# librosa/librosa

Hardware: AMD Instinct MI355X
Metric: STFT+mel frames/sec (n_fft=2048 hop=512) (higher is better)
Workload: dtype f32

## Files before the change

include/librosa_amd.h:

```cpp
#ifndef LIBROSA_AMD_H
#define LIBROSA_AMD_H

#include <stddef.h>
#include <stdint.h>

#ifdef __cplusplus
extern "C" {
#endif

#define LRA_OK 0
#define LRA_EINVAL (-1)
#define LRA_EHIP (-2)
#define LRA_EROCFFT (-3)
#define LRA_ENODEV (-4)
#define LRA_ENOMEM (-5)

#define LRA_F32 0
#define LRA_F64 1

#define LRA_PAD_CONSTANT 0
#define LRA_PAD_REFLECT 1
#define LRA_PAD_EDGE 2
#define LRA_PAD_SYMMETRIC 3

// ... 176 lines not shown
    int halve;
    int64_t n;
    const void* row_ptr;
    const void* col;
    const void* val;
} lra_cqt_octave;
int lra_cqt_recursion_exec(lra_ctx* ctx, const void* y, int64_t batch, const lra_cqt_octave* octaves, int n_octaves, int pad_mode, const void* sqrt_len, void* out, int64_t n_frames,
                           int n_total, const void* taps, int n_taps, int first, void* scratch, int64_t scratch_bytes, int overlap, int dtype);
int lra_cqt_octave_exec(lra_ctx* ctx, const void* y, int64_t batch, int64_t n, int64_t y_stride, int n_fft, int hop, int pad_mode, const void* row_ptr, const void* col, const void* val,
                        const void* sqrt_len, void* out, int64_t n_frames, int n_total, int bin0, int row0, int n_rows, int dtype);

int lra_magnitude_exec(lra_ctx* ctx, const void* D, void* mag, int64_t count, int dtype);

int lra_magphase_exec(lra_ctx* ctx, const void* D, int is_complex, void* mag, void* phase, int64_t count, double power, int dtype);

int lra_hpss_exec(lra_ctx* ctx, const void* mag, const void* D, void* out_h, void* out_p, int64_t batch, int64_t n_frames, int n_bins, int win_harm, int win_perc, double power,
                  double margin_harm, double margin_perc, int want_mask, int dtype);

#define LRA_COMM_ID_BYTES 128
typedef struct lra_comm lra_comm;
int lra_comm_unique_id(void* id_out);
int lra_comm_init(lra_ctx* ctx, int rank, int n_ranks, const void* id, lra_comm** out);
int lra_comm_allgather(lra_comm* comm, const void* send_dev, void* recv_dev, size_t bytes_per_rank);
int lra_comm_allgatherv(lra_comm* comm, const void* send_dev, void* recv_dev, const size_t* bytes_per_rank, const size_t* recv_offsets);
void lra_comm_destroy(lra_comm* comm);

int lra_probe_stream(lra_ctx* ctx, int direction, const void* in, void* out, int64_t batch, int64_t rows_per_clip, int n_fft, int hop, int64_t clip_samples,
                     int strip_rows, int waves_per_cu);
int lra_probe_stream_pitched(lra_ctx* ctx, int direction, const void* in, void* out, int64_t batch, int64_t rows_per_clip, int n_fft, int hop, int64_t clip_samples,
                             int strip_rows, int waves_per_cu, int64_t row_pitch_bytes, int piece_bytes);

int lra_probe_stream_window(lra_ctx* ctx, const void* in, void* out, int64_t batch, int64_t rows_per_clip, int n_fft, int hop, int64_t clip_samples, int strip_rows, int waves_per_cu);

int lra_transpose(lra_ctx* ctx, const void* src, void* dst, int64_t batch, int64_t rows, int64_t cols, int elem_bytes);

#ifdef __cplusplus
}
#endif
#endif
```

librosa_amd/_native.py:

```python
from __future__ import annotations

import collections
import ctypes
import os
import threading
from ctypes import POINTER, byref, c_char_p, c_double, c_float, c_int, c_int64, c_size_t, c_void_p

import numpy as np

from .util.exceptions import LibrosaError, ParameterError

_HERE = os.path.dirname(os.path.abspath(__file__))
LIB_PATH = os.environ.get("LIBROSA_AMD_LIBRARY") or os.path.join(_HERE, "_liblibrosa_amd.so")

LRA_OK, LRA_EINVAL, LRA_EHIP, LRA_EROCFFT, LRA_ENODEV, LRA_ENOMEM = 0, -1, -2, -3, -4, -5
LRA_F32, LRA_F64 = 0, 1
PAD_MODES = {"constant": 0, "reflect": 1, "edge": 2, "symmetric": 3}


class NativeError(LibrosaError):
    """The HIP library is missing, or a HIP / rocFFT call failed."""


SIGNATURES = {
# ... 11 lines not shown
    "lra_ctx_nonfinite_reset": (c_int, [c_void_p]),
    "lra_ctx_nonfinite_read": (c_int, [c_void_p, POINTER(c_int)]),
    "lra_stft_plan_is_fused": (c_int, [c_void_p]),
    "lra_stft_plan_tuned_variant": (c_int, [c_void_p, c_int]),
    "lra_istft_plan_tuned_variant": (c_int, [c_void_p]),
    "lra_malloc": (c_int, [c_void_p, c_size_t, POINTER(c_void_p)]),
    "lra_free": (c_int, [c_void_p, c_void_p]),
    "lra_malloc_placed": (c_int, [c_void_p, c_size_t, c_int, c_int64, c_int, POINTER(c_void_p), POINTER(c_float), POINTER(c_int)]),
    "lra_free_placed": (c_int, [c_void_p, c_void_p]),
    "lra_memset": (c_int, [c_void_p, c_void_p, c_int, c_size_t]),
    "lra_memcpy_h2d": (c_int, [c_void_p, c_void_p, c_void_p, c_size_t]),
    "lra_memcpy_d2h": (c_int, [c_void_p, c_void_p, c_void_p, c_size_t]),
    "lra_event_create": (c_int, [c_void_p, POINTER(c_void_p)]),
    "lra_event_destroy": (None, [c_void_p]),
    "lra_event_record": (c_int, [c_void_p]),
    "lra_event_elapsed_ms": (c_int, [c_void_p, c_void_p, POINTER(c_float)]),
    "lra_stft_plan_create": (c_int, [c_void_p, c_int, c_int, c_void_p, c_int, c_int, c_int, POINTER(c_void_p)]),
    "lra_stft_plan_destroy": (None, [c_void_p]),
    "lra_stft_num_frames": (c_int, [c_void_p, c_int64, POINTER(c_int64)]),
    "lra_stft_exec": (c_int, [c_void_p, c_void_p, c_int64, c_int64, c_int64, c_void_p]),
    "lra_spectrogram_exec": (c_int, [c_void_p, c_void_p, c_int64, c_int64, c_int64, c_double, c_void_p]),
    "lra_mel_plan_create": (c_int, [c_void_p, c_int, c_int, c_void_p, c_int, POINTER(c_void_p)]),
    "lra_mel_plan_destroy": (None, [c_void_p]),
    "lra_melspectrogram_exec": (c_int, [c_void_p, c_void_p, c_void_p, c_int64, c_int64, c_int64, c_double, c_void_p]),
    "lra_mel_apply_exec": (c_int, [c_void_p, c_void_p, c_int64, c_int64, c_int64, c_int64, c_int64, c_void_p]),
    "lra_istft_plan_create": (c_int, [c_void_p, c_int, c_int, c_void_p, c_int, c_int, POINTER(c_void_p)]),
    "lra_istft_plan_destroy": (None, [c_void_p]),
    "lra_istft_exec": (c_int, [c_void_p, c_void_p, c_int64, c_int64, c_int64, c_int64, c_void_p, c_void_p, c_int64, c_int64]),
    "lra_istft_exec_norm": (c_int, [c_void_p, c_void_p, c_int64, c_int64, c_int64, c_int64, c_void_p, c_void_p, c_int64, c_int64]),
    "lra_transpose": (c_int, [c_void_p, c_void_p, c_void_p, c_int64, c_int64, c_int64, c_int]),
    "lra_probe_stream": (c_int, [c_void_p, c_int, c_void_p, c_void_p, c_int64, c_int64, c_int, c_int, c_int64, c_int, c_int]),
    "lra_cqt_recursion_exec": (c_int, [c_void_p, c_void_p, c_int64, c_void_p, c_int, c_int, c_void_p, c_void_p, c_int64, c_int, c_void_p, c_int, c_int, c_void_p, c_int64, c_int, c_int]),
    "lra_probe_stream_window": (c_int, [c_void_p, c_void_p, c_void_p, c_int64, c_int64, c_int, c_int, c_int64, c_int, c_int]),
    "lra_pcg64_random_exec": (c_int, [c_void_p, POINTER(ctypes.c_uint64), ctypes.c_uint64, c_void_p, c_int64]),
    "lra_griffinlim_init_pcg64": (c_int, [c_void_p, POINTER(ctypes.c_uint64), c_void_p, c_void_p, c_int64, c_int, c_int64, c_int]),
    "lra_probe_stream_pitched": (c_int, [c_void_p, c_int, c_void_p, c_void_p, c_int64, c_int64, c_int, c_int, c_int64, c_int, c_int, c_int64, c_int]),
    "lra_stft_exec_strided": (c_int, [c_void_p, c_int, c_void_p, c_int64, c_int64, c_int64, c_double, c_void_p, c_int64]),
    "lra_item_absmax_exec": (c_int, [c_void_p, c_void_p, c_int64, c_int64, c_int, c_void_p]),
    "lra_item_max_exec": (c_int, [c_void_p, c_void_p, c_int64, c_int64, c_int, c_int, c_void_p]),
    "lra_to_db_exec": (c_int, [c_void_p, c_void_p, c_void_p, c_int64, c_int64, c_int, c_int, c_double, c_double, c_void_p, c_void_p, c_int, c_double]),
    "lra_from_db_exec": (c_int, [c_void_p, c_void_p, c_void_p, c_int64, c_int, c_int, c_double]),
    "lra_istft_exec_host": (c_int, [c_void_p, c_void_p, c_int64, c_int64, c_int64, c_void_p, c_void_p, c_int64, c_int64]),
    "lra_stft_exec_host": (c_int, [c_void_p, c_void_p, c_int, c_void_p, c_int64, c_int64, c_int64, c_double, c_void_p, c_int64, POINTER(c_int)]),
    "lra_comm_unique_id": (c_int, [c_void_p]),
    "lra_comm_init": (c_int, [c_void_p, c_int, c_int, c_void_p, POINTER(c_void_p)]),
    "lra_comm_allgather": (c_int, [c_void_p, c_void_p, c_void_p, c_size_t]),
    "lra_comm_allgatherv": (c_int, [c_void_p, c_void_p, c_void_p, POINTER(c_size_t), POINTER(c_size_t)]),
    "lra_comm_destroy": (None, [c_void_p]),
    "lra_phase_vocoder_exec": (c_int, [c_void_p, c_void_p, c_void_p, c_int64, c_int64, c_int, c_void_p, c_int64, c_int]),
    "lra_griffinlim_init": (c_int, [c_void_p, c_void_p, c_void_p, c_void_p, c_int64, c_int]),
    "lra_griffinlim_update": (c_int, [c_void_p, c_void_p, c_void_p, c_void_p, c_void_p, c_int64, c_int, c_double, c_double, c_int]),
    "lra_pcen_exec": (c_int, [c_void_p, c_void_p, c_void_p, c_void_p, c_int64, c_int64, c_int, c_double, c_double, c_double, c_double, c_double, c_void_p, c_double, c_void_p]),
    "lra_maxfilter_exec": (c_int, [c_void_p, c_void_p, c_void_p, c_int64, c_int, c_int64, c_int, c_int]),
    "lra_onset_exec": (c_int, [c_void_p, c_void_p, c_void_p, c_void_p, c_int64, c_int, c_int64, c_int, c_int, c_int, c_int, c_void_p, c_void_p, c_int, c_int, c_int64, c_int64, c_int,
                               c_double, c_double, c_void_p, c_int, c_void_p]),
    "lra_beat_work_bytes": (c_int64, [c_int64, c_int64, c_int]),
    "lra_beat_exec": (c_int, [c_void_p, c_void_p, c_int64, c_int64, c_int, c_void_p, c_int, c_double, c_double, c_int, c_void_p, c_void_p, POINTER(c_int)]),
    "lra_peak_pick_work_bytes": (c_int64, [c_int64, c_int64, c_int]),
    "lra_peak_pick_exec": (c_int, [c_void_p, c_void_p, c_int64, c_int64, c_int, c_int, c_int64, c_int64, c_int64, c_int64, c_double, c_int64, c_int, c_void_p, c_void_p, c_void_p,
                                   POINTER(c_int)]),
    "lra_prev_minimum_exec": (c_int, [c_void_p, c_void_p, c_int64, c_int64, c_int, c_void_p]),
    "lra_tempogram_work_bytes": (c_int64, [c_int64, c_int64, c_int, c_int]),
    "lra_tempogram_exec": (c_int, [c_void_p, c_void_p, c_int64, c_int64, c_int, c_int, c_int, c_void_p, c_int, c_int, c_void_p, c_void_p, c_void_p, c_void_p, POINTER(c_int)]),
    "lra_fir_decimate_exec": (c_int, [c_void_p, c_void_p, c_void_p, c_int64, c_int64, c_int64, c_void_p, c_int, c_int, c_int, c_double, c_double, c_int]),
    "lra_resample_poly_exec": (c_int, [c_void_p, c_void_p, c_void_p, c_int64, c_int64, c_int64, c_void_p, c_int, c_int, c_int, c_int, c_double, c_double, c_int]),
    "lra_resample_fft_exec": (c_int, [c_void_p, c_void_p, c_void_p, c_int64, c_int64, c_int64, c_double, c_int]),
# ... 626 lines not shown
```

librosa_amd/csrc/lra_api.hip:

```cpp
#include <dlfcn.h>
#include <hip/hip_runtime.h>
#include <rocfft/rocfft.h>

#include <algorithm>
#include <atomic>
#include <chrono>
#include <cmath>
#include <cstdio>
#include <cstdlib>
#include <cstring>
#include <map>
#include <memory>
#include <mutex>
#include <string>
#include <thread>
#include <vector>

#include "../../include/librosa_amd.h"
#define LRA_FUSED_EXTERN
#include "lra_fused.h"
#include "lra_mel.h"
#include "lra_post.h"
#include "lra_pcen.h"
#include "lra_onset.h"
// ... 368 lines not shown
                const double fill = (v2 && Cfg::TF == 64 && rounds <= 1.0 && rounds >= 0.6) ? 1.0 : rounds / std::ceil(rounds);
                if (fill > best_fill + 0.02) { best_fill = fill; best_iters = it; }
            }
            iters = best_iters;
            while (iters > 4 && batch * ((a.n_frames + fpb * iters - 1) / (fpb * iters)) < 2LL * n_cu) iters /= 2;
        }
        if (iters < 1) iters = 1;
        a.rot_uniform = 0;
        if (Cfg::FPB > 1 && Cfg::TF < 64 && ring_rows_aligned<Cfg>(a.hop)) {
            if (iters_opt <= 0 && iters >= 4) iters = (iters + 3) / 4 * 4;
            a.rot_uniform = iters % 4 == 0;
        }
        a.mel_tile = mel_tile_opt > 0 ? mel_tile_opt : 4;
        if (a.mel_tile > iters) a.mel_tile = iters;
        a.frames_per_wg = Cfg::FPB * iters;
        a.wg_per_clip = (a.n_frames + a.frames_per_wg - 1) / a.frames_per_wg;
        a.slot_bytes = v2 ? stft2_slot_bytes<Cfg>() : direct ? Cfg::FRAME_BYTES : stft_slot_bytes<Cfg>(MODE, a.n_mels, a.mel_tile);
        a.shared_off = Cfg::FPB * a.slot_bytes;
        const long long grid = batch * a.wg_per_clip;
        if (grid > 0x7ffffff0LL) { err = hipErrorInvalidConfiguration; return; }
        const int lds = Cfg::FPB * a.slot_bytes + shared_bytes + lds_pad;
        if (lds > 160 * 1024) { err = hipErrorInvalidValue; return; }
        if (lds > 65536) {
            err = hipFuncSetAttribute(reinterpret_cast<const void*>(kern), hipFuncAttributeMaxDynamicSharedMemorySize, lds);
            if (err != hipSuccess) return;
        }
        a.n_blocks = (int)grid;
        a.xcd_chunk = (xcd_remap && grid >= 64) ? (int)((grid + 7) / 8) : 0;
        const long long launch_grid = a.xcd_chunk ? 8LL * a.xcd_chunk : grid;
        hipLaunchKernelGGL(kern, dim3((unsigned)launch_grid), dim3(Cfg::NT), lds, stream, a, a.y, out);
        err = hipGetLastError();
    }

    template <class Cfg> void launch_pc(int hd) {
        using PL = PcLayout<Cfg>;
        void (*kern)(StftArgs<T>, const T*, void*) = nullptr;
#define LRA_PICKP(HD)                                                        \
    kern = stft_pc_kernel<Cfg, HD, POW_TWO>;                                 \
    if (a.power_mode == POW_ONE) kern = stft_pc_kernel<Cfg, HD, POW_ONE>;    \
    if (a.power_mode == POW_GENERAL) kern = stft_pc_kernel<Cfg, HD, POW_GENERAL>;
        if (hd == 4) { LRA_PICKP(4) } else { LRA_PICKP(8) }
#undef LRA_PICKP
        const int lds = PL::BYTES + lds_pad;
        constexpr int fpb = PL::NP;
        int iters = iters_opt;
        if (iters <= 0) {
            const int per_cu = resident_workgroups(reinterpret_cast<const void*>(kern), PL::NT, lds);
            const long long conc = (long long)n_cu * (per_cu > 0 ? per_cu : 1);
            int best_iters = 0;
            double best_fill = -1.0;
            for (int cand = 176; cand >= 24; --cand) {
                const int wgpc = (a.n_frames + fpb * cand - 1) / (fpb * cand);
                const int it = (a.n_frames + fpb * wgpc - 1) / (fpb * wgpc);
                const double rounds = (double)(batch * wgpc) / (double)conc;
                const double fill = (rounds <= 1.0 && rounds >= 0.6) ? 1.0 : rounds / std::ceil(rounds);
                if (fill > best_fill + 0.02) { best_fill = fill; best_iters = it; }
            }
            iters = best_iters;
            while (iters > 4 && batch * ((a.n_frames + fpb * iters - 1) / (fpb * iters)) < 2LL * n_cu) iters /= 2;
        }
        if (iters < 1) iters = 1;
        a.rot_uniform = 0;
        a.mel_tile = 1;
        a.frames_per_wg = fpb * iters;
        a.wg_per_clip = (a.n_frames + a.frames_per_wg - 1) / a.frames_per_wg;
        a.slot_bytes = PL::FRAME;
        a.shared_off = 0;
        const long long grid = batch * a.wg_per_clip;
        if (grid > 0x7ffffff0LL) { err = hipErrorInvalidConfiguration; return; }
        a.n_blocks = (int)grid;
        a.xcd_chunk = (xcd_remap && grid >= 64) ? (int)((grid + 7) / 8) : 0;
        const long long launch_grid = a.xcd_chunk ? 8LL * a.xcd_chunk : grid;
        hipLaunchKernelGGL(kern, dim3((unsigned)launch_grid), dim3(PL::NT), lds, stream, a, a.y, out);
        err = hipGetLastError();
    }

    template <class Cfg> void operator()() {
        if constexpr (Cfg::REV) {
            err = hipErrorInvalidValue;
            return;
        } else if constexpr (Cfg::PLAN == 1) {
            if (!use_v2 || v2_hop_divisor<Cfg>(a.hop) == 0) { err = hipErrorInvalidValue; return; }
            if (mode == OUT_COMPLEX) launch<Cfg, OUT_COMPLEX>(0);
            else if (mode == OUT_POWER) launch<Cfg, OUT_POWER>(0);
            else if (mode == OUT_MEL2 && mel_pc && mel && mel->melr2_ok && mel_runs) {
                if constexpr (pc_cfg_ok<Cfg>()) {
                    const int hd_pc = v2_hop_divisor<Cfg>(a.hop);
                    if (!pc_bank_ok<Cfg>(a.n_mels, mel->melr2_pmax) || !pc_fits_budget<Cfg>(hd_pc, a.power_mode)) { err = hipErrorInvalidValue; return; }
                    a.melr_w = (const T*)mel->d_melr2_w;
                    a.melr_keep = (const T*)mel->d_melr2_keep;
                    a.melr_addr = mel->d_melr2_addr;
                    a.melr_zero = mel->melr2_zero;
                    a.melr_mid = mel->melr2_mid;
                    a.melr_pmax = mel->melr2_pmax;
                    launch_pc<Cfg>(hd_pc);
                } else err = hipErrorInvalidValue;
            } else err = hipErrorInvalidValue;
        } else {
            run<Cfg>();
        }
    }
    template <class Cfg> void run() {
        if (mode == OUT_MEL2) {
            using MC = typename MelCfgOf<Cfg>::type;
            if constexpr (pc_cfg_ok<Cfg>()) {
                const int hd_pc = v2_hop_divisor<Cfg>(a.hop);
                if (mel_pc && mel && mel->melr2_ok && mel_runs && use_v2 && pc_bank_ok<Cfg>(a.n_mels, mel->melr2_pmax) && pc_fits_budget<Cfg>(hd_pc, a.power_mode)) {
                    a.melr_w = (const T*)mel->d_melr2_w;
                    a.melr_keep = (const T*)mel->d_melr2_keep;
                    a.melr_addr = mel->d_melr2_addr;
                    a.melr_zero = mel->melr2_zero;
                    a.melr_mid = mel->melr2_mid;
                    a.melr_pmax = mel->melr2_pmax;
                    launch_pc<Cfg>(hd_pc);
                    return;
                }
            }
            if constexpr (v2_cfg_ok<MC>()) {
                if (mel && mel->melr2_ok && mel_runs && use_v2 && melr_fits<MC>() && v2_hop_divisor<MC>(a.hop) > 0) {
                    const int shared_r = melr_shared_bytes<MC>(a.n_mels, mel->melr2_pmax);
                    if (MC::FPB * stft2_slot_bytes<MC>() + shared_r <= 160 * 1024) {
                        a.melr_w = (const T*)mel->d_melr2_w;
                        a.melr_keep = (const T*)mel->d_melr2_keep;
                        a.melr_addr = mel->d_melr2_addr;
                        a.melr_zero = mel->melr2_zero;
                        a.melr_mid = mel->melr2_mid;
                        a.melr_pmax = mel->melr2_pmax;
                        mel_v2 = true;
                        mel_tile_opt = 1;
                        launch<MC, OUT_MELR>(shared_r);
                        return;
                    }
                }
            }
            if constexpr (mel_many_applies<Cfg>()) {
                using MM = typename MelManyCfgOf<Cfg>::type;
                if (mel && mel->melr_ok && mel->melr_many && mel_runs && melr_fits<MM>()) {
                    const int shared_m = melr_shared_bytes<MM>(a.n_mels, mel->melr_pmax);
                    if (MM::FPB * stft_slot_bytes<MM>(OUT_MELR, a.n_mels, 1) + shared_m <= 160 * 1024) {
                        a.melr_w = (const T*)mel->d_melr_w;
                        a.melr_keep = (const T*)mel->d_melr_keep;
                        a.melr_addr = mel->d_melr_addr;
                        a.melr_zero = mel->melr_zero;
                        a.melr_mid = mel->melr_mid;
                        a.melr_pmax = mel->melr_pmax;
                        mel_tile_opt = 1;
                        launch<MM, OUT_MELR>(shared_m);
                        return;
// ... 3234 lines not shown
    if (n_fft < 256 || n_fft > 2048 || M % 128 != 0) return fail(LRA_EINVAL, "probe: n_fft must be 256 ... 2048, a multiple of 256");
    if (hop <= 0 || hop > 1024 || hop % 128 != 0) return fail(LRA_EINVAL, "probe: hop must be a multiple of 128, at most 1024");
    if (direction != 0 && direction != 1) return fail(LRA_EINVAL, "probe: direction 0 (forward stream) or 1 (inverse stream)");
    if (rows_per_clip > 0x7fffffffLL || batch > 0x7fffffffLL) return fail(LRA_EINVAL, "probe: too many rows");
    ProbeArgs a;
    a.in = (const char*)in;
    a.out = (char*)out;
    a.clip_in_bytes = (long long)clip_samples * 4;
    a.rows_per_clip = (int)rows_per_clip;
    a.strip_rows = strip_rows > 0 ? strip_rows : 162;
    a.n_clips = (int)batch;
    a.bins = M + 1;
    a.row_pitch = row_pitch_bytes > 0 ? row_pitch_bytes : (long long)(M + 1) * 8;
    if (a.row_pitch < (long long)(M + 1) * 8 || a.row_pitch % 8 != 0) return fail(LRA_EINVAL, "probe: row pitch must be a multiple of 8 bytes, at least one row");
    if (piece_bytes != 8 && piece_bytes != 16) return fail(LRA_EINVAL, "probe: pieces of 8 or 16 bytes");
    if (piece_bytes == 16 && (a.row_pitch % 16 != 0 || ((size_t)(direction == 0 ? out : in) & 15))) return fail(LRA_EINVAL, "probe: 16-byte pieces need 16-byte aligned rows");
    a.hop_bytes = hop * 4;
    const long long pcm_rows = clip_samples / hop;
    a.pcm_rows = (int)(pcm_rows < rows_per_clip ? pcm_rows : rows_per_clip);
    const long long strips = (long long)batch * ((rows_per_clip + a.strip_rows - 1) / a.strip_rows);
    const long long grid = (strips + 7) / 8 * 8;
    if (grid > 0x7ffffff0LL) return fail(LRA_EINVAL, "probe: grid too large");
    a.xcd_chunk = ctx->opt_xcd_remap ? (int)(grid / 8) : 0;
    const int wpc = waves_per_cu > 0 ? waves_per_cu : 12;
    const int lds = wpc >= 32 ? 0 : ((160 * 1024 / wpc) & ~255);
    auto kern = direction == 0 ? (piece_bytes == 16 ? stream_probe_kernel<0, true> : stream_probe_kernel<0, false>)
                               : (piece_bytes == 16 ? stream_probe_kernel<1, true> : stream_probe_kernel<1, false>);
    if (lds > 65536) LRA_HIP(hipFuncSetAttribute(reinterpret_cast<const void*>(kern), hipFuncAttributeMaxDynamicSharedMemorySize, lds));
    hipLaunchKernelGGL(kern, dim3((unsigned)grid), dim3(64), lds, ctx->stream, a);
    LRA_HIP(hipGetLastError());
    return LRA_OK;
}

int lra_probe_stream_window(lra_ctx* ctx, const void* in, void* out, int64_t batch, int64_t rows_per_clip, int n_fft, int hop, int64_t clip_samples, int strip_rows, int waves_per_cu) {
    LRA_BIND(ctx);
    if (batch <= 0 || rows_per_clip <= 0) return LRA_OK;
    if (!in || !out) return fail(LRA_EINVAL, "null data pointer");
    const int M = n_fft / 2;
    if (n_fft < 256 || n_fft > 2048 || M % 128 != 0) return fail(LRA_EINVAL, "probe: n_fft must be 256 ... 2048, a multiple of 256");
    if (hop <= 0 || hop > 1024 || hop % 128 != 0) return fail(LRA_EINVAL, "probe: hop must be a multiple of 128, at most 1024");
    if (strip_rows < 1 || waves_per_cu < 1 || waves_per_cu > 32) return fail(LRA_EINVAL, "probe: strip_rows >= 1, 1 <= waves_per_cu <= 32");
    ProbeArgs a;
    a.in = (const char*)in;
    a.out = (char*)out;
    a.clip_in_bytes = (long long)clip_samples * 4;
    a.rows_per_clip = (int)rows_per_clip;
    a.strip_rows = strip_rows;
    a.n_clips = (int)batch;
    a.bins = M + 1;
    a.row_pitch = (long long)(M + 1) * 8;
    a.hop_bytes = hop * 4;
    const long long pcm_rows = clip_samples / hop;
    a.pcm_rows = (int)(pcm_rows < rows_per_clip ? pcm_rows : rows_per_clip);
    a.xcd_chunk = 0;
    const int n_workers = ctx->n_cu * waves_per_cu;
    const int lds = waves_per_cu >= 32 ? 0 : ((160 * 1024 / waves_per_cu) & ~255);
    if (lds > 65536) LRA_HIP(hipFuncSetAttribute(reinterpret_cast<const void*>(stream_probe_window_kernel), hipFuncAttributeMaxDynamicSharedMemorySize, lds));
    hipLaunchKernelGGL(stream_probe_window_kernel, dim3((unsigned)n_workers), dim3(64), lds, ctx->stream, a, (long long)batch * rows_per_clip, n_workers);
    LRA_HIP(hipGetLastError());
    return LRA_OK;
}

int lra_transpose(lra_ctx* ctx, const void* src, void* dst, int64_t batch, int64_t rows, int64_t cols, int elem_bytes) {
    LRA_BIND(ctx);
    if (batch <= 0 || rows <= 0 || cols <= 0) return LRA_OK;
    if (!src || !dst) return fail(LRA_EINVAL, "null data pointer");
// ... 15 lines not shown
```

librosa_amd/csrc/lra_fused.h:

```cpp
#pragma once

#include <hip/hip_runtime.h>

#include "lra_dispatch.h"
#include "lra_kernels_pc.h"

template <class Cfg, int MODE, int PM, int RA>
__global__ __launch_bounds__(Cfg::NT, Cfg::MIN_WAVES) void stft_kernel(lra::StftArgs<typename Cfg::real> a, const typename Cfg::real* __restrict__ y,
                                                                     void* __restrict__ out) {
    extern __shared__ __attribute__((aligned(16))) char lra_smem[];
    lra::Lds lds;
    lds.base = lra_smem;
    a.y = y;
    a.D = static_cast<typename Cfg::cplx*>(out);
    a.S = static_cast<typename Cfg::real*>(out);
    a.Mel = static_cast<typename Cfg::real*>(out);
    const int blk = lra::xcd_block((int)blockIdx.x, a.xcd_chunk);
    if (blk >= a.n_blocks) return;
    lra::stft_block<Cfg, MODE, PM, RA>(a, blk, lds);
}

constexpr int kV3Waves = 3;
template <class Cfg, int HD, int MODE, int PM>
__global__ __launch_bounds__(Cfg::NT, (Cfg::NT > 256 ? 1 : (Cfg::TF == 64 && HD >= 4 && PM != lra::POW_GENERAL && MODE != lra::OUT_MELR ? (Cfg::PLAN == 1 ? kV3Waves : 3) : 2))) void stft2_kernel(lra::StftArgs<typename Cfg::real> a, const typename Cfg::real* __restrict__ y,
                                                                                  void* __restrict__ out) {
    extern __shared__ __attribute__((aligned(16))) char lra_smem[];
    lra::Lds lds;
    lds.base = lra_smem;
    a.y = y;
    a.D = static_cast<typename Cfg::cplx*>(out);
    a.S = static_cast<typename Cfg::real*>(out);
    a.Mel = static_cast<typename Cfg::real*>(out);
    const int blk = lra::xcd_block((int)blockIdx.x, a.xcd_chunk);
    if (blk >= a.n_blocks) return;
    lra::stft_block2<Cfg, HD, MODE, PM>(a, blk, lds);
}

template <class Cfg, int HD, int PM>
__global__ __launch_bounds__(lra::PcLayout<Cfg>::NT, 3) void stft_pc_kernel(lra::StftArgs<typename Cfg::real> a, const typename Cfg::real* __restrict__ y, void* __restrict__ out) {
    extern __shared__ __attribute__((aligned(32))) char lra_smem[];
    lra::Lds lds;
    lds.base = lra_smem;
    a.y = y;
    a.Mel = static_cast<typename Cfg::real*>(out);
    const int blk = lra::xcd_block((int)blockIdx.x, a.xcd_chunk);
    if (blk >= a.n_blocks) return;
    lra::stft_pc_block<Cfg, HD, PM>(a, blk, lds);
}

template <class Cfg, int HC>
__global__ __launch_bounds__(Cfg::NT, Cfg::MIN_WAVES) void istft_kernel(lra::IstftArgs<typename Cfg::real> a, const typename Cfg::cplx* __restrict__ D,
                                                                      const typename Cfg::real* __restrict__ wss, typename Cfg::real* __restrict__ y) {
    extern __shared__ __attribute__((aligned(16))) char lra_smem[];
    lra::Lds lds;
    lds.base = lra_smem;
    a.D = D;
    a.wss = wss;
    a.y = y;
    const int blk = lra::xcd_block((int)blockIdx.x, a.xcd_chunk);
    if (blk >= a.n_blocks) return;
    lra::istft_block<Cfg, HC>(a, blk, lds);
}


namespace lra {

#define LRA_CFG_ALIAS(NAME, ...) using NAME = typename CfgSel<__VA_ARGS__>::type; using NAME##_mel = typename MelCfgOf<NAME>::type; using NAME##_melmany = typename MelManyCfgOf<NAME>::type;
LRA_CFG_ALIAS(cfg_f32_4, float, 4, 0)
LRA_CFG_ALIAS(cfg_f32_5, float, 5, 0)
LRA_CFG_ALIAS(cfg_f32_6, float, 6, 0)
LRA_CFG_ALIAS(cfg_f32_7, float, 7, 0)
LRA_CFG_ALIAS(cfg_f32_8, float, 8, 0)
LRA_CFG_ALIAS(cfg_f32_9, float, 9, 0)
LRA_CFG_ALIAS(cfg_f32_10, float, 10, 0)
LRA_CFG_ALIAS(cfg_f32_10v1, float, 10, 1)
LRA_CFG_ALIAS(cfg_f32_10v4, float, 10, 4)
LRA_CFG_ALIAS(cfg_f32_10r, float, 10, 5)
LRA_CFG_ALIAS(cfg_f32_10g, float, 10, 6)
LRA_CFG_ALIAS(cfg_f32_10q, float, 10, 7)
LRA_CFG_ALIAS(cfg_f32_11, float, 11, 0)
// ... 74 lines not shown
```

librosa_amd/csrc/lra_kernels_pc.h:

```cpp
#pragma once

#include "lra_kernels2.h"

namespace lra {

constexpr int kPcPrioPA = 3, kPcPrioPS = 2, kPcPrioCA = 0, kPcPrioCB = 1;
constexpr int kPcSpinLimit = 1 << 22;

template <class Cfg> struct PcLayout {
    using T = typename Cfg::real;
    static constexpr int NP = 2;
    static constexpr int NT = (NP + 1) * Cfg::TF;
    static constexpr int FRAME = Cfg::FRAME_BYTES;
    static constexpr int PW = (v2_pw_bytes<Cfg>() + 15) / 16 * 16;
    static constexpr int RS = ((Cfg::R * (Cfg::TF + kMelRsPitchExtra) + 2) * 2 * (int)sizeof(T) + 15) / 16 * 16;
    static constexpr int frame_off(int s) { return s * FRAME; }
    static constexpr int pw_off(int s) { return NP * FRAME + s * PW; }
    static constexpr int rs_off() { return NP * (FRAME + PW); }
    static constexpr int flags_off() { return rs_off() + RS; }
    static constexpr int ready_off(int s) { return flags_off() + 4 * s; }
    static constexpr int consumed_off(int s) { return flags_off() + 4 * (NP + s); }
    static constexpr int BYTES = flags_off() + 16;
};

template <class Cfg> constexpr bool pc_cfg_ok() { return v23_cfg_ok<Cfg>() && Cfg::TF == 64 && v2_pw_swz<Cfg>() && melr_fits<Cfg>() && sizeof(typename Cfg::real) == 4; }
template <class Cfg> LRA_HD bool pc_bank_ok(int n_mels, int pmax) { return n_mels >= 1 && n_mels <= 2 * Cfg::TF && pmax <= 4; }

template <class Cfg> LRA_HD bool pc_fits_budget(int hd, int power_mode) {
    if (power_mode != POW_TWO && power_mode != POW_ONE) return false;
    if (hd == 8) return true;
    return hd == 4 && (power_mode == POW_TWO || Cfg::PLAN == 1);
}

#ifdef LRA_HOSTSIM
struct PcTileV {
    float e[16];
    float& operator[](int i) { return e[i]; }
    float operator[](int i) const { return e[i]; }
};
#else
typedef float PcTileV __attribute__((ext_vector_type(16)));
#endif

template <class Cfg> struct PcRegs {
    using T = typename Cfg::real;
    using C = typename Cfg::cplx;
    static constexpr int NB = 2, PH = 4, TILE = 8, NP = PcLayout<Cfg>::NP;
    C w[Cfg::R];
    C wq;
    T keep[Cfg::R];
    T pw[Cfg::R], pw_extra;
    int mad[NB][2 * PH];
    int pwa[4], pwx;
    T* row[NB];
    int ph[NP][NB];
    PcTileV mt[NP];
// ... 15 lines not shown
}
#endif
template <class T, int MT> LRA_HD void pc_tile_band(const PcTileV& t, int b, T (&out)[MT]) {
    LRA_UNROLL
    for (int k = 0; k < MT; ++k) out[k] = t[MT * b + k];
}

#ifdef LRA_HOSTSIM
LRA_HD int pc_flag_load(Lds l, int off) { return lds_ld<int>(l, off); }
LRA_HD void pc_flag_store(Lds l, int off, int v) { lds_st<int>(l, off, v); }
LRA_HD void pc_wait(Lds, int, int, unsigned int*) {}
LRA_HD void pc_fence() {}
#else
__device__ __forceinline__ void pc_fence() {
    __builtin_amdgcn_fence(__ATOMIC_RELEASE, "wavefront");
    __builtin_amdgcn_wave_barrier();
    __builtin_amdgcn_fence(__ATOMIC_ACQUIRE, "wavefront");
}
__device__ __forceinline__ int pc_flag_load(Lds l, int off) { return *(const volatile __attribute__((address_space(3))) int*)(l.base + off); }
__device__ __forceinline__ void pc_flag_store(Lds l, int off, int v) { *(volatile __attribute__((address_space(3))) int*)(l.base + off) = v; }
__device__ __forceinline__ void pc_wait(Lds l, int off, int want, unsigned int* sticky) {
    int spins = 0;
    while (true) {
        const int v = LRA_UNIFORM(pc_flag_load(l, off));
        if (LRA_LIKELY(v >= want)) break;
        if (LRA_UNLIKELY(++spins > kPcSpinLimit)) {
            if (sticky && (threadIdx.x & 63) == 0) atomicOr(sticky, 2u);
            break;
        }
        __builtin_amdgcn_s_sleep(2);
    }
    pc_fence();
}
__device__ __forceinline__ void pc_wait_ready(Lds l, int off, int want, unsigned int* sticky) {
    if (LRA_UNLIKELY(LRA_UNIFORM(pc_flag_load(l, off)) < want)) pc_wait(l, off, want, sticky);
    else pc_fence();
}
#endif

template <class Cfg, int HD> LRA_HD void pc_producer_prologue(const StftArgs<typename Cfg::real>& a, int clip, int frame0, int tf, Regs2<Cfg, HD>& rg) {
    using T = typename Cfg::real;
    if constexpr (Cfg::PLAN == 1) v3_hoist<Cfg, HD>(rg, tf, a.win, a.tw, a.twr);
    else v2_hoist<Cfg, HD>(rg, tf, a.win, a.tw, a.twr);
    v2_fill<Cfg, HD>(a, clip, frame0, tf, rg);
    if constexpr (v2_rotate_asm_ok<Cfg, HD>()) {
        LRA_UNROLL
        for (int e = 0; e < Cfg::R; ++e) { LRA_KEEP(rg.raw[e].x); LRA_KEEP(rg.raw[e].y); }
    }
    LRA_UNROLL
    for (int e = 0; e < Regs2<Cfg, HD>::NEW; ++e) rg.pf[e] = mk<T>((T)0, (T)0);
}
template <class Cfg, int HD> LRA_HD void pc_producer_pass0(const StftArgs<typename Cfg::real>& a, int clip, int frame, int it, bool more, int tf, Regs2<Cfg, HD>& rg, Lds fr) {
    if (v2_rotate_asm_ok<Cfg, HD>()) {
        v2_window_rotating<Cfg, HD>(it, rg);
        if (more) v2_issue_loads<Cfg, HD>(a, clip, frame + 1, tf, rg);
        v2_pass0_dft<Cfg, HD>(tf, rg, fr);
    } else {
        if (it > 0) v2_shift<Cfg, HD>(rg);
        if (more) v2_issue_loads<Cfg, HD>(a, clip, frame + 1, tf, rg);
        v2_pass0<Cfg, HD>(frame < a.n_frames, tf, rg, fr);
    }
}

template <class Cfg, int p> LRA_HD void pc_mid_dft_write(typename Cfg::cplx* v, const typename Cfg::cplx* treg, Lds fr, int tf) {
    if constexpr (Cfg::PLAN == 1) {
        v3_mid_twiddle_dft<Cfg>(v, treg);
        v3_mid_write<Cfg>(v, fr, tf);
    } else {
// ... 113 lines not shown
        for (int h = 0; h < 2; ++h) {
            T acc = (T)0;
            LRA_UNROLL
            for (int q = 0; q < PH; ++q) acc += x[b][h * PH + q];
            part[h] = acc;
        }
        const T v = part[0] + part[1];
        int s8;
        if constexpr (UNI) {
            s8 = (rg.ph[S][b] + it) & (MT - 1);
            mt[MT * b + s8] = v;
        } else {
            s8 = (int)((rg.row[b] - a.Mel + frame) & (MT - 1));
            LRA_UNROLL
            for (int k = 0; k < MT; ++k) mt[MT * b + k] = k == s8 ? v : mt[MT * b + k];
        }
        if (last_of_slot || s8 == MT - 1) {
            T t8[MT];
            pc_tile_band(mt, b, t8);
            melr_burst_row(rg.row[b] + (frame - s8), s8, it, t8);
        }
    }
    return mt;
}

#ifndef LRA_HOSTSIM
template <class Cfg, bool UNI> __device__ __forceinline__ void pc_consumer(const StftArgs<typename Cfg::real>& a, int clip, int f_first, int iters, int n_it, Lds lds) {
    using L = PcLayout<Cfg>;
    constexpr int TF = Cfg::TF;
    PcRegs<Cfg> rg;
    const Lds rs = lds_sub(lds, L::rs_off());
    const int tf = (int)(threadIdx.x & (TF - 1));
    pc_consumer_prologue<Cfg>(a, clip, f_first, iters, tf, rg, lds);
    pc_fence();
    for (int it = 0; it < n_it; ++it) {
#define LRA_PC_SERVE(S)                                                                                                        \
        {                                                                                                                      \
            const int frame = f_first + S * iters + it;                                                                       \
            v2_setprio<kPcPrioCA>();                                                                                      \
            pc_wait_ready(lds, L::ready_off(S), it + 1, a.nonfinite_flag);                                                     \
            pc_runs_read<Cfg>(rg, lds_sub(lds, L::pw_off(S)));                                                                 \
            pc_fence();                                                                                                        \
            if (tf == 0) pc_flag_store(lds, L::consumed_off(S), it + 1);                             \
            pc_fence();                                                                                                        \
            pc_accumulate<Cfg>(a, tf, rg, rs);                                                                                 \
            pc_fence();                                                                                                        \
            v2_setprio<kPcPrioCB>();                                                                                      \
            if (frame < a.n_frames) rg.mt[S] = pc_combine<Cfg, S, UNI>(a, clip, frame, tf, it, it + 1 == iters || frame + 1 >= a.n_frames, rg, lds, rg.mt[S]); \
            pc_fence();                                                                                                        \
        }
        LRA_PC_SERVE(0)
        LRA_PC_SERVE(1)
#undef LRA_PC_SERVE
    }
}
#endif

template <class Cfg, int HD, int PM = POW_TWO> LRA_HD void stft_pc_block(const StftArgs<typename Cfg::real>& a_in, const int blk, Lds lds) {
    static_assert(pc_cfg_ok<Cfg>(), "producer / consumer mel kernel: one wave per frame, mirrored last pass, swizzled power row");
    using T = typename Cfg::real;
    using L = PcLayout<Cfg>;
    using RG = Regs2<Cfg, HD>;
    constexpr int NP = L::NP, TF = Cfg::TF;
    StftArgs<T> a = a_in;
    const int clip = blk / a.wg_per_clip;
    const int f_first = (blk % a.wg_per_clip) * a.frames_per_wg;
    const int iters = a.frames_per_wg / NP;
    const int left = a.n_frames - f_first;
    const int n_it = left < iters ? left : iters;
#ifdef LRA_HOSTSIM
    LRA_REGS(RG, prg, L::NT);
    LRA_REGS(PcRegs<Cfg>, crg, L::NT);
    LRA_PHASE(L::NT, tid) {
        const int w = tid / TF, tf = tid % TF;
        if (w < NP) pc_producer_prologue<Cfg, HD>(a, clip, f_first + w * iters, tf, LRA_R(prg));
        else pc_consumer_prologue<Cfg>(a, clip, f_first, iters, tf, LRA_R(crg), lds);
        if (tid < 2 * NP) pc_flag_store(lds, L::flags_off() + 4 * tid, 0);
    } LRA_PHASE_END
    for (int it = 0; it < n_it; ++it) {
        LRA_PHASE(L::NT, tid) {
            const int w = tid / TF, tf = tid % TF;
            if (w < NP) pc_producer_pass0<Cfg, HD>(a, clip, f_first + w * iters + it, it, it + 1 < iters, tf, LRA_R(prg), lds_sub(lds, L::frame_off(w)));
        } LRA_PHASE_END_SYNC(true)
#define LRA_PC_MID(p)                                                                                                                   \
        if (Cfg::P - 1 > p) {                                                                                                           \
            LRA_PHASE(L::NT, tid) {                                                                                                     \
                if (tid / TF < NP) pass_read<Cfg, (p < Cfg::P ? p : 0)>(LRA_R(prg).v, lds_sub(lds, L::frame_off(tid / TF)), tid % TF);  \
            } LRA_PHASE_END_SYNC(true)                                                                                                  \
            LRA_PHASE(L::NT, tid) {                                                                                                     \
                if (tid / TF < NP) pc_mid_dft_write<Cfg, (p < Cfg::P ? p : 0)>(LRA_R(prg).v, LRA_R(prg).treg, lds_sub(lds, L::frame_off(tid / TF)), tid % TF); \
            } LRA_PHASE_END_SYNC(true)                                                                                                  \
// ... 3 lines not shown
#undef LRA_PC_MID
        LRA_PHASE(L::NT, tid) {
            if (tid / TF < NP) pc_last_read<Cfg, HD>(LRA_R(prg), lds_sub(lds, L::frame_off(tid / TF)), tid % TF);
        } LRA_PHASE_END_SYNC(true)
        LRA_PHASE(L::NT, tid) {
            const int w = tid / TF, tf = tid % TF, frame = f_first + w * iters + it;
            if (w < NP) pc_last_power_row<Cfg, HD, PM>(a, clip, frame, tf, LRA_R(prg), lds_sub(lds, L::pw_off(w)));
        } LRA_PHASE_END
        for (int s = 0; s < NP; ++s) {
            LRA_PHASE(L::NT, tid) {
                if (tid / TF == NP) pc_runs_read<Cfg>(LRA_R(crg), lds_sub(lds, L::pw_off(s)));
            } LRA_PHASE_END_SYNC(true)
            LRA_PHASE(L::NT, tid) {
                if (tid / TF == NP) pc_accumulate<Cfg>(a, tid % TF, LRA_R(crg), lds_sub(lds, L::rs_off()));
            } LRA_PHASE_END_SYNC(true)
            LRA_PHASE(L::NT, tid) {
                const int tf = tid % TF, frame = f_first + s * iters + it;
                if (tid / TF == NP && frame < a.n_frames) {
                    const bool last = it + 1 == iters || frame + 1 >= a.n_frames;
                    if (pc_tile_uniform<Cfg>(a)) {
                        if (s == 0) LRA_R(crg).mt[0] = pc_combine<Cfg, 0, true>(a, clip, frame, tf, it, last, LRA_R(crg), lds, LRA_R(crg).mt[0]);
                        else LRA_R(crg).mt[1] = pc_combine<Cfg, 1, true>(a, clip, frame, tf, it, last, LRA_R(crg), lds, LRA_R(crg).mt[1]);
                    } else {
                        if (s == 0) LRA_R(crg).mt[0] = pc_combine<Cfg, 0, false>(a, clip, frame, tf, it, last, LRA_R(crg), lds, LRA_R(crg).mt[0]);
                        else LRA_R(crg).mt[1] = pc_combine<Cfg, 1, false>(a, clip, frame, tf, it, last, LRA_R(crg), lds, LRA_R(crg).mt[1]);
                    }
                }
            } LRA_PHASE_END_SYNC(true)
        }
        sim::state().barrier();
    }
#else
    static_assert((TF & (TF - 1)) == 0 && L::pw_off(0) % 32 == 0 && L::PW % 32 == 0, "lane mask; power rows start on 32 bytes (v2_pw_addr_xor)");
    if (threadIdx.x < 2 * NP) pc_flag_store(lds, L::flags_off() + 4 * (int)threadIdx.x, 0);
    phase_sync<false>();
    const int wave = LRA_UNIFORM((int)(threadIdx.x / TF));
    if (wave < NP) {
        RG rg;
        const Lds fr = lds_sub(lds, L::frame_off(wave)), pwr = lds_sub(lds, L::pw_off(wave));
        {
            const int tf = (phase_tid() & (TF - 1));
            pc_producer_prologue<Cfg, HD>(a, clip, f_first + wave * iters, tf, rg);
        }
        pc_fence();
        for (int it = 0; it < n_it; ++it) {
            const int frame = f_first + wave * iters + it;
            v2_setprio<kPcPrioPA>();
            {
                const int tf = (phase_tid() & (TF - 1));
                pc_producer_pass0<Cfg, HD>(a, clip, frame, it, it + 1 < iters, tf, rg, fr);
            }
            pc_fence();
#define LRA_PC_MID(p)                                                                                    \
            if (Cfg::P - 1 > p) {                                                                        \
                { const int tf = (phase_tid() & (TF - 1)); pass_read<Cfg, (p < Cfg::P ? p : 0)>(rg.v, fr, tf); } \
                pc_fence();                                                                              \
                { const int tf = (phase_tid() & (TF - 1)); pc_mid_dft_write<Cfg, (p < Cfg::P ? p : 0)>(rg.v, rg.treg, fr, tf); } \
                pc_fence();                                                                              \
            }
            LRA_PC_MID(1)
            LRA_PC_MID(2)
#undef LRA_PC_MID
            int taken;
            {
                const int tf = (phase_tid() & (TF - 1));
                pc_last_read<Cfg, HD>(rg, fr, tf);
                taken = pc_flag_load(lds, L::consumed_off(wave));
            }
            pc_fence();
            v2_setprio<kPcPrioPS>();
            if (LRA_UNLIKELY(LRA_UNIFORM(taken) < it)) pc_wait(lds, L::consumed_off(wave), it, a.nonfinite_flag);
            {
                const int tf = (phase_tid() & (TF - 1));
                pc_last_power_row<Cfg, HD, PM>(a, clip, frame, tf, rg, pwr);
            }
            pc_fence();
            if ((phase_tid() & (TF - 1)) == 0) pc_flag_store(lds, L::ready_off(wave), it + 1);
            pc_fence();
        }
    } else {
        if (pc_tile_uniform<Cfg>(a)) pc_consumer<Cfg, true>(a, clip, f_first, iters, n_it, lds);
        else pc_consumer<Cfg, false>(a, clip, f_first, iters, n_it, lds);
    }
#endif
}

}
```

Before: 649.3 million.

## Pack four producer/consumer wave trios into one workgroup for the STFT+mel kernel

The producer/consumer mel kernel now launches workgroups containing four independent trios (two producer waves plus one consumer), each with its own LDS slice. Block indices are mapped per trio, and the XCD remap is applied to groups. This is meant to cut workgroup launch overhead and the per-workgroup residency limits, so more trios stay resident per CU. It also moves the consumed-flag load ahead of the last read and uses precomputed flag addresses. The cost is larger LDS per workgroup, with a fallback when it exceeds 160KB. Idle trios in a partial group exit after the barrier.

After: 648.3 million. About the same (-0.1%).

```diff
diff --git a/include/librosa_amd.h b/include/librosa_amd.h
--- a/include/librosa_amd.h
+++ b/include/librosa_amd.h
@@ -232,6 +232,8 @@
 
 int lra_probe_stream_window(lra_ctx* ctx, const void* in, void* out, int64_t batch, int64_t rows_per_clip, int n_fft, int hop, int64_t clip_samples, int strip_rows, int waves_per_cu);
 
+int lra_pc_group_map(int blocks, int xcd_remap, int* n_workgroups, int* map, int64_t cap);
+
 int lra_transpose(lra_ctx* ctx, const void* src, void* dst, int64_t batch, int64_t rows, int64_t cols, int elem_bytes);
 
 #ifdef __cplusplus
diff --git a/librosa_amd/_native.py b/librosa_amd/_native.py
--- a/librosa_amd/_native.py
+++ b/librosa_amd/_native.py
@@ -67,6 +67,7 @@
     "lra_probe_stream": (c_int, [c_void_p, c_int, c_void_p, c_void_p, c_int64, c_int64, c_int, c_int, c_int64, c_int, c_int]),
     "lra_cqt_recursion_exec": (c_int, [c_void_p, c_void_p, c_int64, c_void_p, c_int, c_int, c_void_p, c_void_p, c_int64, c_int, c_void_p, c_int, c_int, c_void_p, c_int64, c_int, c_int]),
     "lra_probe_stream_window": (c_int, [c_void_p, c_void_p, c_void_p, c_int64, c_int64, c_int, c_int, c_int64, c_int, c_int]),
+    "lra_pc_group_map": (c_int, [c_int, c_int, POINTER(c_int), POINTER(c_int), c_int64]),
     "lra_pcg64_random_exec": (c_int, [c_void_p, POINTER(ctypes.c_uint64), ctypes.c_uint64, c_void_p, c_int64]),
     "lra_griffinlim_init_pcg64": (c_int, [c_void_p, POINTER(ctypes.c_uint64), c_void_p, c_void_p, c_int64, c_int, c_int64, c_int]),
     "lra_probe_stream_pitched": (c_int, [c_void_p, c_int, c_void_p, c_void_p, c_int64, c_int64, c_int, c_int, c_int64, c_int, c_int, c_int64, c_int]),
diff --git a/librosa_amd/csrc/lra_api.hip b/librosa_amd/csrc/lra_api.hip
--- a/librosa_amd/csrc/lra_api.hip
+++ b/librosa_amd/csrc/lra_api.hip
@@ -424,7 +424,7 @@
         err = hipGetLastError();
     }
 
-    template <class Cfg> void launch_pc(int hd) {
+    template <class Cfg> bool launch_pc(int hd) {
         using PL = PcLayout<Cfg>;
         void (*kern)(StftArgs<T>, const T*, void*) = nullptr;
 #define LRA_PICKP(HD)                                                        \
@@ -433,12 +433,14 @@
     if (a.power_mode == POW_GENERAL) kern = stft_pc_kernel<Cfg, HD, POW_GENERAL>;
         if (hd == 4) { LRA_PICKP(4) } else { LRA_PICKP(8) }
 #undef LRA_PICKP
-        const int lds = PL::BYTES + lds_pad;
+        const int lds = kPcGroup * PL::BYTES + lds_pad;
+        if (lds > 160 * 1024) return false;
+        const int per_cu = resident_workgroups(reinterpret_cast<const void*>(kern), kPcGroup * PL::NT, lds);
+        if (per_cu < 1) return false;
         constexpr int fpb = PL::NP;
         int iters = iters_opt;
         if (iters <= 0) {
-            const int per_cu = resident_workgroups(reinterpret_cast<const void*>(kern), PL::NT, lds);
-            const long long conc = (long long)n_cu * (per_cu > 0 ? per_cu : 1);
+            const long long conc = (long long)n_cu * kPcGroup * per_cu;
             int best_iters = 0;
             double best_fill = -1.0;
             for (int cand = 176; cand >= 24; --cand) {
@@ -459,12 +461,12 @@
         a.slot_bytes = PL::FRAME;
         a.shared_off = 0;
         const long long grid = batch * a.wg_per_clip;
-        if (grid > 0x7ffffff0LL) { err = hipErrorInvalidConfiguration; return; }
+        if (grid > 0x7fffff00LL) { err = hipErrorInvalidConfiguration; return true; }
         a.n_blocks = (int)grid;
-        a.xcd_chunk = (xcd_remap && grid >= 64) ? (int)((grid + 7) / 8) : 0;
-        const long long launch_grid = a.xcd_chunk ? 8LL * a.xcd_chunk : grid;
-        hipLaunchKernelGGL(kern, dim3((unsigned)launch_grid), dim3(PL::NT), lds, stream, a, a.y, out);
+        a.xcd_chunk = pc_xcd_chunk(a.n_blocks, xcd_remap);
+        hipLaunchKernelGGL(kern, dim3((unsigned)pc_launch_grid(a.n_blocks, xcd_remap)), dim3(kPcGroup * PL::NT), lds, stream, a, a.y, out);
         err = hipGetLastError();
+        return true;
     }
 
     template <class Cfg> void operator()() {
@@ -485,7 +487,7 @@
                     a.melr_zero = mel->melr2_zero;
                     a.melr_mid = mel->melr2_mid;
                     a.melr_pmax = mel->melr2_pmax;
-                    launch_pc<Cfg>(hd_pc);
+                    if (!launch_pc<Cfg>(hd_pc)) err = hipErrorInvalidValue;
                 } else err = hipErrorInvalidValue;
             } else err = hipErrorInvalidValue;
         } else {
@@ -504,8 +506,7 @@
                     a.melr_zero = mel->melr2_zero;
                     a.melr_mid = mel->melr2_mid;
                     a.melr_pmax = mel->melr2_pmax;
-                    launch_pc<Cfg>(hd_pc);
-                    return;
+                    if (launch_pc<Cfg>(hd_pc)) return;
                 }
             }
             if constexpr (v2_cfg_ok<MC>()) {
@@ -3806,6 +3807,20 @@
     return LRA_OK;
 }
 
+int lra_pc_group_map(int blocks, int xcd_remap, int* n_workgroups, int* map, int64_t cap) {
+    if (blocks < 0 || blocks > 0x7fffff00 || !n_workgroups) return fail(LRA_EINVAL, "pc group map: bad block count or null count");
+    const int chunk = pc_xcd_chunk(blocks, xcd_remap != 0), grid = pc_launch_grid(blocks, xcd_remap != 0);
+    *n_workgroups = grid;
+    if (!map || cap < (int64_t)kPcGroup * grid) return fail(LRA_EINVAL, "pc group map: map too small");
+    for (int wg = 0; wg < grid; ++wg) {
+        for (int w = 0; w < kPcGroup * 3; ++w) {
+            const int t = pc_wave_trio(w), blk = pc_group_block(wg, t, chunk);
+            map[kPcGroup * wg + t] = blk < blocks ? blk : -1;
+        }
+    }
+    return LRA_OK;
+}
+
 int lra_probe_stream_window(lra_ctx* ctx, const void* in, void* out, int64_t batch, int64_t rows_per_clip, int n_fft, int hop, int64_t clip_samples, int strip_rows, int waves_per_cu) {
     LRA_BIND(ctx);
     if (batch <= 0 || rows_per_clip <= 0) return LRA_OK;
diff --git a/librosa_amd/csrc/lra_fused.h b/librosa_amd/csrc/lra_fused.h
--- a/librosa_amd/csrc/lra_fused.h
+++ b/librosa_amd/csrc/lra_fused.h
@@ -37,15 +37,16 @@
 }
 
 template <class Cfg, int HD, int PM>
-__global__ __launch_bounds__(lra::PcLayout<Cfg>::NT, 3) void stft_pc_kernel(lra::StftArgs<typename Cfg::real> a, const typename Cfg::real* __restrict__ y, void* __restrict__ out) {
+__global__ __launch_bounds__(lra::kPcGroup * lra::PcLayout<Cfg>::NT, 3) void stft_pc_kernel(lra::StftArgs<typename Cfg::real> a, const typename Cfg::real* __restrict__ y, void* __restrict__ out) {
     extern __shared__ __attribute__((aligned(32))) char lra_smem[];
-    lra::Lds lds;
-    lds.base = lra_smem;
     a.y = y;
     a.Mel = static_cast<typename Cfg::real*>(out);
-    const int blk = lra::xcd_block((int)blockIdx.x, a.xcd_chunk);
-    if (blk >= a.n_blocks) return;
-    lra::stft_pc_block<Cfg, HD, PM>(a, blk, lds);
+    const int w = LRA_UNIFORM((int)(threadIdx.x / Cfg::TF));
+    const int trio = lra::pc_wave_trio(w);
+    lra::Lds lds;
+    lds.base = lra_smem + trio * lra::PcLayout<Cfg>::BYTES;
+    const int blk = lra::pc_group_block((int)blockIdx.x, trio, a.xcd_chunk);
+    lra::stft_pc_block<Cfg, HD, PM>(a, blk, lds, lra::pc_wave_role(w), blk < a.n_blocks);
 }
 
 template <class Cfg, int HC>
diff --git a/librosa_amd/csrc/lra_kernels_pc.h b/librosa_amd/csrc/lra_kernels_pc.h
--- a/librosa_amd/csrc/lra_kernels_pc.h
+++ b/librosa_amd/csrc/lra_kernels_pc.h
@@ -20,8 +20,16 @@
     static constexpr int flags_off() { return rs_off() + RS; }
     static constexpr int ready_off(int s) { return flags_off() + 4 * s; }
     static constexpr int consumed_off(int s) { return flags_off() + 4 * (NP + s); }
-    static constexpr int BYTES = flags_off() + 16;
+    static constexpr int BYTES = (flags_off() + 16 + 31) / 32 * 32;
 };
+
+constexpr int kPcGroup = 4;
+LRA_HD int pc_wave_trio(int w) { return w / 3; }
+LRA_HD int pc_wave_role(int w) { return w % 3; }
+LRA_HD int pc_groups(int blocks) { return (blocks + kPcGroup - 1) / kPcGroup; }
+LRA_HD int pc_xcd_chunk(int blocks, bool remap) { return (remap && blocks >= 64) ? (pc_groups(blocks) + 7) / 8 : 0; }
+LRA_HD int pc_launch_grid(int blocks, bool remap) { const int chunk = pc_xcd_chunk(blocks, remap); return chunk ? 8 * chunk : pc_groups(blocks); }
+LRA_HD int pc_group_block(int wg, int trio, int xcd_chunk) { return kPcGroup * xcd_block(wg, xcd_chunk) + trio; }
 
 template <class Cfg> constexpr bool pc_cfg_ok() { return v23_cfg_ok<Cfg>() && Cfg::TF == 64 && v2_pw_swz<Cfg>() && melr_fits<Cfg>() && sizeof(typename Cfg::real) == 4; }
 template <class Cfg> LRA_HD bool pc_bank_ok(int n_mels, int pmax) { return n_mels >= 1 && n_mels <= 2 * Cfg::TF && pmax <= 4; }
@@ -103,8 +111,23 @@
     }
     pc_fence();
 }
-__device__ __forceinline__ void pc_wait_ready(Lds l, int off, int want, unsigned int* sticky) {
-    if (LRA_UNLIKELY(LRA_UNIFORM(pc_flag_load(l, off)) < want)) pc_wait(l, off, want, sticky);
+__device__ __forceinline__ int pc_flag_load_at(int fl, int off) { return *(const volatile __attribute__((address_space(3))) int*)(size_t)(unsigned int)(fl + off); }
+__device__ __forceinline__ void pc_flag_store_at(int fl, int off, int v) { *(volatile __attribute__((address_space(3))) int*)(size_t)(unsigned int)(fl + off) = v; }
+__device__ __forceinline__ void pc_wait_at(int fl, int rel, int want, unsigned int* sticky) {
+    int spins = 0;
+    while (true) {
+        const int v = LRA_UNIFORM(pc_flag_load_at(fl, rel));
+        if (LRA_LIKELY(v >= want)) break;
+        if (LRA_UNLIKELY(++spins > kPcSpinLimit)) {
+            if (sticky && (threadIdx.x & 63) == 0) atomicOr(sticky, 2u);
+            break;
+        }
+        __builtin_amdgcn_s_sleep(2);
+    }
+    pc_fence();
+}
+__device__ __forceinline__ void pc_wait_ready(int fl, int rel, int want, unsigned int* sticky) {
+    if (LRA_UNLIKELY(LRA_UNIFORM(pc_flag_load_at(fl, rel)) < want)) pc_wait_at(fl, rel, want, sticky);
     else pc_fence();
 }
 #endif
@@ -284,16 +307,17 @@
     const Lds rs = lds_sub(lds, L::rs_off());
     const int tf = (int)(threadIdx.x & (TF - 1));
     pc_consumer_prologue<Cfg>(a, clip, f_first, iters, tf, rg, lds);
+    const int fl = pc_mad_addr(lds, L::flags_off());
     pc_fence();
     for (int it = 0; it < n_it; ++it) {
 #define LRA_PC_SERVE(S)                                                                                                        \
         {                                                                                                                      \
             const int frame = f_first + S * iters + it;                                                                       \
             v2_setprio<kPcPrioCA>();                                                                                      \
-            pc_wait_ready(lds, L::ready_off(S), it + 1, a.nonfinite_flag);                                                     \
+            pc_wait_ready(fl, L::ready_off(S) - L::flags_off(), it + 1, a.nonfinite_flag);                                     \
             pc_runs_read<Cfg>(rg, lds_sub(lds, L::pw_off(S)));                                                                 \
             pc_fence();                                                                                                        \
-            if (tf == 0) pc_flag_store(lds, L::consumed_off(S), it + 1);                             \
+            if (tf == 0) pc_flag_store_at(fl, L::consumed_off(S) - L::flags_off(), it + 1);          \
             pc_fence();                                                                                                        \
             pc_accumulate<Cfg>(a, tf, rg, rs);                                                                                 \
             pc_fence();                                                                                                        \
@@ -308,7 +332,7 @@
 }
 #endif
 
-template <class Cfg, int HD, int PM = POW_TWO> LRA_HD void stft_pc_block(const StftArgs<typename Cfg::real>& a_in, const int blk, Lds lds) {
+template <class Cfg, int HD, int PM = POW_TWO> LRA_HD void stft_pc_block(const StftArgs<typename Cfg::real>& a_in, const int blk, Lds lds, const int role = 0, const bool live = true) {
     static_assert(pc_cfg_ok<Cfg>(), "producer / consumer mel kernel: one wave per frame, mirrored last pass, swizzled power row");
     using T = typename Cfg::real;
     using L = PcLayout<Cfg>;
@@ -378,9 +402,14 @@
     }
 #else
     static_assert((TF & (TF - 1)) == 0 && L::pw_off(0) % 32 == 0 && L::PW % 32 == 0, "lane mask; power rows start on 32 bytes (v2_pw_addr_xor)");
-    if (threadIdx.x < 2 * NP) pc_flag_store(lds, L::flags_off() + 4 * (int)threadIdx.x, 0);
+    static_assert(L::BYTES % 32 == 0, "every trio's slice starts on 32 bytes");
+    {
+        const int tl = (int)(threadIdx.x % (unsigned)L::NT);
+        if (tl < 2 * NP) pc_flag_store(lds, L::flags_off() + 4 * tl, 0);
+    }
     phase_sync<false>();
-    const int wave = LRA_UNIFORM((int)(threadIdx.x / TF));
+    if (!live) return;
+    const int wave = role;
     if (wave < NP) {
         RG rg;
         const Lds fr = lds_sub(lds, L::frame_off(wave)), pwr = lds_sub(lds, L::pw_off(wave));
@@ -410,8 +439,8 @@
             int taken;
             {
                 const int tf = (phase_tid() & (TF - 1));
+                taken = pc_flag_load(lds, L::consumed_off(wave));
                 pc_last_read<Cfg, HD>(rg, fr, tf);
-                taken = pc_flag_load(lds, L::consumed_off(wave));
             }
             pc_fence();
             v2_setprio<kPcPrioPS>();
```
